# rgcgithub/regenie

Hardware: NVIDIA H100
Metric: step1_level0_snps_per_sec (higher is better)
Workload: dtype int8 Gram + int8 prediction (both exact integer sums) + tf32x3 factorisation + f64 refinement / statistics

## Files before the change

regenie_b200/csrc/bed_kernels.cu:

```cuda
#include "kernels.cuh"

namespace rg {

__device__ __forceinline__ uint32_t plink_to_code(uint32_t v, int ref_first) {
  const uint32_t lut = ref_first ? 0x9Cu : 0x1Eu;
  return (lut >> (2 * v)) & 3u;
}

__global__ void bed_relayout_kernel(const uint8_t* __restrict__ packed, int64_t row_stride, int bs,
                                    const int32_t* __restrict__ file_idx_pad, const int32_t* __restrict__ word_base,
                                    const uint32_t* __restrict__ word_keep, int ref_first,
                                    uint32_t* __restrict__ gp, int64_t words_per_row) {
  const int64_t w = blockIdx.x * (int64_t)blockDim.x + threadIdx.x;
  const int row = blockIdx.y;
  if (w >= words_per_row) return;
  uint32_t out = 0;
  const int base = (row < bs) ? __ldg(word_base + w) : -1;
  if (base >= 0) {
    const uint8_t* p = packed + (int64_t)row * row_stride + (base >> 2);
    const int64_t left = row_stride - (base >> 2);
    uint64_t x = 0;
#pragma unroll
    for (int b = 0; b < 5; ++b)
      if (b < left) x |= (uint64_t)__ldg(p + b) << (8 * b);
    const uint32_t v = (uint32_t)(x >> (2 * (base & 3)));
    const uint32_t H = (v >> 1) & 0x55555555u, Lo = v & 0x55555555u;
    const uint32_t oh = ref_first ? Lo : (~H & 0x55555555u);
    out = ((oh << 1) | (H ^ Lo)) & __ldg(word_keep + w);
  } else if (base == -2) {
    const uint8_t* prow = packed + (int64_t)row * row_stride;
    const int4* fi4 = reinterpret_cast<const int4*>(file_idx_pad + w * 16);
#pragma unroll
    for (int q = 0; q < 4; ++q) {
      const int4 f = __ldg(fi4 + q);
      const int fi[4] = {f.x, f.y, f.z, f.w};
#pragma unroll
      for (int k = 0; k < 4; ++k) {
        uint32_t code = 0;
        if (fi[k] >= 0) {
          const uint32_t b = __ldg(prow + (fi[k] >> 2));
          code = plink_to_code((b >> (2 * (fi[k] & 3))) & 3u, ref_first);
        }
        out |= code << (2 * (q * 4 + k));
      }
    }
  }
  gp[(int64_t)row * words_per_row + w] = out;
}

void launch_bed_relayout(const uint8_t* packed, int64_t row_stride, int bs, int rows_p,
                         const int32_t* file_idx_pad, const int32_t* word_base, const uint32_t* word_keep, int ref_first,
                         uint32_t* gp, int64_t npad,
                         cudaStream_t s) {
  const int64_t wpr = npad / 16;
  dim3 grid((unsigned)ceil_div(wpr, 256), rows_p);
  bed_relayout_kernel<<<grid, 256, 0, s>>>(packed, row_stride, bs, file_idx_pad, word_base, word_keep, ref_first, gp, wpr);
}

}
```

regenie_b200/csrc/context.cuh:

```cuda
#pragma once
#include <map>
#include <memory>

#include "../../include/rg_b200.h"
#include "kernels.cuh"

struct rg_ctx;
namespace rg { void ensure_W(::rg_ctx* h); }

struct rg_ctx {
  int kind = 0;
  int device = 0;
  cudaStream_t stream = nullptr;
  int64_t launches = 0;

  int64_t N = 0, Npad = 0, n_analyzed = 0;
  int C = 0, P = 0, K = 1, R = 0, R1 = 0, loocv = 0;
  int bs_max = 0, rows_p_max = 0, total_blocks = 0, cpp = 0;
  int64_t B = 0;

  std::vector<int64_t> fold_sizes, fold_pad_start, fold_pad_len;
  std::vector<int32_t> pad_of;
  std::vector<int32_t> src_of;
  std::vector<uint8_t> in_analysis;
// ... 127 lines not shown
  rg::DevBuf<double> s2_male_tot;
  int bt_mode = 0, bt_dp = 0, bt_ncol = 0;
  int s2_fcols = 0;
  bool s2_chr_set = false, bt_chr_set = false;
  int s2_last_bs = 0;
  int s2_sums_rows = 0, bt_sums_rows = 0, bt_sums_dp = 0;
  static constexpr int kStageSlots = 4;
  rg::DevBuf<uint8_t> s2_stage[kStageSlots];
  cudaStream_t s2_copy_stream = nullptr;
  cudaEvent_t s2_stage_ev[kStageSlots] = {nullptr, nullptr, nullptr, nullptr};
  bool s2_stage_pending[kStageSlots] = {false, false, false, false};
  rg::DevBuf<uint8_t> probs_dev, miss_dev;
  rg::DevBuf<uint8_t> inflate_comp, inflate_raw;
  rg::DevBuf<uint64_t> inflate_offs;
  rg::DevBuf<int32_t> inflate_status;
  rg::DevBuf<uint8_t> pgen_in, pgen_rows;
  rg::DevBuf<unsigned long long> pgen_err;
  rg::DevBuf<uint32_t> dz;
  bool int_set = false;
  bool s2_dz_qt = false;
  rg::DevBuf<int8_t> int_route;
  int int_K = 0, int_nr = 0, int_nf = 0;
  rg::DevBuf<double> int_F, int_E, int_part, int_sums, int_var, int_meat, int_out;
  rg::DevBuf<uint8_t> int_pow2;
  rg::DevBuf<int32_t> int_status;
  rg::DevBuf<double> bt_F, bt_w, bt_gs, bt_xw, bt_off, bt_coltot, bt_xwy, bt_part, bt_sums, bt_nnz, bt_n510;
  rg::DevBuf<double> bt_xtwg, bt_mu, bt_info, firth_gvec, firth_out, bt_den, bt_phat;
  rg::DevBuf<int8_t> bt_ym, firth_cflag;
  rg::DevBuf<int2> bt_cnt_part;
  rg::DevBuf<int32_t> firth_sel, firth_status;

  bool gram_dense = false;
  int64_t miss_cap = 0;

  int solver_mixed = 1;
  float mx_tol = 1e-9f;
  int64_t mx_blocks = 0, mx_fallbacks = 0;

  bool timing = false;
  cudaEvent_t ev0 = nullptr, ev1 = nullptr;
  std::map<std::string, std::pair<double, int64_t>> timers;
  std::vector<std::tuple<std::string, cudaEvent_t, cudaEvent_t>> pending;
};

namespace rg {
void require_gpu(int device);
void ensure_file_idx(rg_ctx* h, const int32_t* sample_idx);
void flush_timers(rg_ctx* h);
void sync_lanes(rg_ctx* h);
void pgen_check_errors(rg_ctx* h);
}

#define RG_API_BEGIN try {
#define RG_API_END                         \
  }                                        \
  catch (const rg::Error& e) {             \
    rg::set_last_error(e.msg);             \
    return 1;                              \
  }                                        \
  catch (const std::exception& e) {        \
    rg::set_last_error(e.what());          \
    return 1;                              \
  }                                        \
  return 0;
```

regenie_b200/csrc/kernels.cuh:

```cuda
#pragma once
#include "common.cuh"

namespace rg {

constexpr int kMaxFolds = 16;
constexpr int kMaxCov = 64;
constexpr int kMaxRidge = 8;
constexpr int kMaxPhenoTile = 8;
constexpr int kLimbs = 9;
constexpr int kLimbsI8 = 5;
constexpr int kLimbQI8 = 50;

void launch_bed_relayout(const uint8_t* packed, int64_t row_stride, int bs, int rows_p,
                         const int32_t* file_idx_pad, const int32_t* word_base, const uint32_t* word_keep, int ref_first,
                         uint32_t* gp, int64_t npad,
                         cudaStream_t s);

struct SnpFinalizeArgs {
  int bs, rows_p, C, P, K, cpp, loocv;
  long long n_analyzed;
  double numtol;
  const int32_t* cnt_fold;
  const double* sum_fold;
  const double* XtX_f;
  const double* XtY_f;
  double *mu, *inv_sd;
  double* Bv;
  double *Af, *Qf;
  double *gty_f, *rhs;
  unsigned long long* err_slot;
  long long err_base;
};

struct AssembleArgs {
  int bs, rows_p, nC, C, K, R, loocv;
  const float* zz;
  int64_t ldz, zz_fold_stride;
  const double *mu, *inv_sd, *Bv, *Af, *Qf;
  const double* lambda;
  double* cm;
  int64_t cm_stride;
  int ldc;
  float* planes = nullptr;
  float* lplanes = nullptr;
};

void launch_l0_stats(const uint32_t* gp, int64_t npad, const double* xy, int cpp, const int4* chunks,
                     int nchunks, int rows_p, int32_t* cnt_part, double* sum_part, cudaStream_t s);
void launch_l0_fold_reduce(const int32_t* cnt_part, const double* sum_part, int rows_p, int cpp,
                           const int2* fold_chunks, int K, int32_t* cnt_fold, double* sum_fold,
                           cudaStream_t s);
void launch_l0_snp_finalize(const SnpFinalizeArgs& a, cudaStream_t s);
void launch_l0_assemble(const AssembleArgs& a, const double* rhs, int P, int Ppad, int nmat, cudaStream_t s);

void make_gram_tensor_map(CUtensorMap* tm, const uint8_t* z, int64_t npad, int rows2);
constexpr int kStatQ = 14;
constexpr int kStatOnesRow = 126;
void launch_l0_xy_digits(const double* xy, int cpp, int ncol, int64_t npad, const uint8_t* is_real, double* scale,
                         uint8_t* D, cudaStream_t s);
void launch_l0_stats_finish(const float* T, int ldt, int64_t t_fold_stride, const float* zz, int ldz,
                            int64_t zz_fold_stride, int rows_p, int cpp, int ncol, int K, const double* scale,
                            int32_t* cnt_fold, double* sum_fold, cudaStream_t s);
void gram_tile_list(int rows2, std::vector<int2>& tiles);
void launch_gram_wgmma(const CUtensorMap& tm, const CUtensorMap& tmB, const int2* tiles, int ntiles, const int2* fold_k, int K,
                         float* out, int ldo, int64_t fold_stride, float out_scale, cudaStream_t s, int bn = 256);
void launch_gram_gp(const CUtensorMap& tmG, const CUtensorMap* tmD, int rows_p, const int2* tiles, int ntiles,
                    const int2* fold_k, int K, float* out, int ldo, int64_t fold_stride, float out_scale, cudaStream_t s,
                    int bn = 256, const unsigned long long* miss_total = nullptr, int64_t miss_cap = 0,
                    int miss_tile0 = 0);
constexpr float kZScaleGram = 1.f / 64;
constexpr float kZScaleStat = 1.f / 8;
constexpr double kMissSparseRate = 0.015;
void launch_miss_list(const uint32_t* gp, int64_t npad, int rows_p, const int2* fold_k, int K, unsigned long long* total,
                      int64_t cap, int2* seg, int32_t* list, cudaStream_t s);
void launch_miss_transpose(const uint32_t* gp, int64_t npad, int rows_p, const unsigned long long* total, int64_t cap,
                           uint32_t* gt, cudaStream_t s);
void launch_miss_sparse(const uint32_t* gt, int rows_p, const int2* seg, const int32_t* list, int K,
                        const unsigned long long* total, int64_t cap, float* zz, int64_t fold_stride, cudaStream_t s);
void launch_gram_reference(const uint32_t* gp, int64_t npad, int rows_p, int k0, int k1, float* out, int ldo,
                           cudaStream_t s);

void launch_chol_factor(double* cm, int64_t stride, int nC, int n_aug, int batch, double* inv,
                        unsigned long long* err_slot, long long err_base, cudaStream_t s);
void launch_chol_backsolve(double* cm, int64_t stride, int nC, int P, int batch, const double* inv,
                           cudaStream_t s);
int chol_num_launches(int nC);
size_t chol_inv_elems(int nC, int batch);
void launch_chol_rows_backsolve(double* cm, int64_t stride, int nC, int row0, int nrows, int batch,
                                const double* inv, cudaStream_t s);

struct Tf32GemmEpilogue {
  int n;
  int64_t out_mat_stride;
  float* out;
  int mirror;
  int b_cols_local;
  int negate;
  int lower_only;
  const double* cin;
  int64_t cin_mat_stride;
  int cin_ld, cin_mat_div;
  const double* diag_add;
  int diag_mod;
  int c_chunks;
  int c_mat_div;
};
void make_tf32_operand_tensor_map(CUtensorMap* tm, const float* base, int cols, int rows, int batch);
void make_f32_rows_tensor_map(CUtensorMap* tm, const float* base, int cols, int64_t rows, int box_cols, int box_rows);
void launch_tf32x3_gemm(const CUtensorMap& tmA, const CUtensorMap& tmB, const int4* tiles, int ntiles, int batch,
                        const Tf32GemmEpilogue& ep, cudaStream_t s, const CUtensorMap* tmC = nullptr);

// ... 239 lines not shown
```

regenie_b200/csrc/miss_gram.cu:

```cuda
#include "kernels.cuh"

namespace rg {

namespace {

__device__ __forceinline__ uint32_t miss_bits(uint32_t w) { return w & (w >> 1) & 0x55555555u; }

constexpr int kListThreads = 256;
constexpr int kChunkWords = 64;
constexpr int kSparseWarps = 4;
constexpr int kCodeStride = kChunkWords + 1;

}

__global__ void __launch_bounds__(kListThreads)
miss_list_kernel(const uint32_t* __restrict__ gp, int64_t wpr, int rows_p, const int2* __restrict__ fold_k,
                 unsigned long long* __restrict__ total, unsigned long long cap, int2* __restrict__ seg,
                 int32_t* __restrict__ list) {
  const int i = blockIdx.x, f = blockIdx.y;
  const int2 fk = fold_k[f];
  const int64_t w0 = (int64_t)fk.x * (kSamplePad / 16), w1 = (int64_t)(fk.x + fk.y) * (kSamplePad / 16);
  const uint32_t* row = gp + (int64_t)i * wpr;
  __shared__ int warp_cnt[kListThreads / 32];
  __shared__ unsigned long long base_s;
  __shared__ int pos_s;
  int n = 0;
  for (int64_t w = w0 + threadIdx.x; w < w1; w += kListThreads) n += __popc(miss_bits(__ldg(row + w)));
#pragma unroll
  for (int o = 16; o > 0; o >>= 1) n += __shfl_xor_sync(0xffffffffu, n, o);
  if ((threadIdx.x & 31) == 0) warp_cnt[threadIdx.x >> 5] = n;
  __syncthreads();
  if (threadIdx.x == 0) {
    int cnt = 0;
    for (int k = 0; k < kListThreads / 32; ++k) cnt += warp_cnt[k];
    const unsigned long long base = cnt ? atomicAdd(total, (unsigned long long)cnt) : 0ull;
    seg[(int64_t)f * rows_p + i] = make_int2((int)(base + cnt <= cap ? base : 0), base + cnt <= cap ? cnt : 0);
    base_s = base + cnt <= cap ? base : ~0ull;
    pos_s = 0;
  }
  __syncthreads();
  const unsigned long long base = base_s;
  if (base == ~0ull) return;
  for (int64_t w = w0 + threadIdx.x; w < w1; w += kListThreads) {
    uint32_t m = miss_bits(__ldg(row + w));
    if (!m) continue;
    int p = atomicAdd(&pos_s, __popc(m));
    for (; m; m &= m - 1) list[base + p++] = (int32_t)(w * 16 + (__ffs(m) - 1) / 2);
  }
}

__global__ void __launch_bounds__(256)
miss_transpose_kernel(const uint32_t* __restrict__ gp, int64_t wpr, int rows_p,
                      const unsigned long long* __restrict__ total, unsigned long long cap, uint32_t* __restrict__ gt) {
  if (*total > cap) return;
  __shared__ uint32_t t[128][33];
  const int64_t wb = (int64_t)blockIdx.x * 32;
  const int r0 = blockIdx.y * 128;
  for (int k = threadIdx.x; k < 128 * 32; k += 256) {
    const int r = k >> 5, c = k & 31;
    t[r][c] = (wb + c < wpr) ? __ldg(gp + (int64_t)(r0 + r) * wpr + wb + c) : 0u;
  }
  __syncthreads();
  const int gw = rows_p / 16;
#pragma unroll
  for (int q = 0; q < 2; ++q) {
    const int sl = threadIdx.x + 256 * q;
    const int c = sl >> 4, sh = 2 * (sl & 15);
    if (wb + c >= wpr) continue;
    uint32_t o[8];
#pragma unroll
    for (int jw = 0; jw < 8; ++jw) {
      uint32_t v = 0;
#pragma unroll
      for (int r = 0; r < 16; ++r) v |= ((t[jw * 16 + r][c] >> sh) & 3u) << (2 * r);
      o[jw] = v;
    }
    uint4* dst = reinterpret_cast<uint4*>(gt + (wb * 16 + sl) * gw + blockIdx.y * 8);
    dst[0] = make_uint4(o[0], o[1], o[2], o[3]);
    dst[1] = make_uint4(o[4], o[5], o[6], o[7]);
  }
}

__global__ void __launch_bounds__(32 * kSparseWarps)
miss_sparse_kernel(const uint32_t* __restrict__ gt, int rows_p, const int2* __restrict__ seg,
                   const int32_t* __restrict__ list, const unsigned long long* __restrict__ total,
                   unsigned long long cap, float* __restrict__ zz, int64_t fold_stride) {
  if (*total > cap) return;
  __shared__ uint32_t acc_s[kSparseWarps][2][16 * kCodeStride];
  __shared__ int smp_s[kSparseWarps][128];
  const int warp = threadIdx.x >> 5, lane = threadIdx.x & 31;
  const int i = blockIdx.x * kSparseWarps + warp, f = blockIdx.y;
  uint32_t* sG = acc_s[warp][0];
  uint32_t* sM = acc_s[warp][1];
  int* sSmp = smp_s[warp];
  const int2 sg = seg[(int64_t)f * rows_p + i];
  const int32_t* lst = list + sg.x;
  const int cnt = sg.y;
  const int gw = rows_p / 16;
  const int r = rows_p + i;
  const int colmax = min(2 * rows_p, 256 * ((r / 128) / 2 + 1));
  float* out = zz + (int64_t)f * fold_stride + (int64_t)r * (2 * rows_p);
  constexpr int off[4] = {0, 2, 1, 3};

  for (int w0 = 0; w0 < gw; w0 += kChunkWords) {
    for (int k = lane; k < 16 * kCodeStride; k += 32) { sG[k] = 0; sM[k] = 0; }
    __syncwarp();
    for (int b0 = 0; b0 < cnt; b0 += 126) {
      const int n = min(cnt - b0, 126);
#pragma unroll
      for (int k = 0; k < 4; ++k) sSmp[32 * k + lane] = 32 * k + lane < n ? __ldg(lst + b0 + 32 * k + lane) : -1;
      __syncwarp();
      uint32_t g8[2][4] = {}, m8[2][4] = {};
      for (int g0 = 0; g0 < n; g0 += 7) {
        uint32_t g4[2][2] = {}, m4[2][2] = {};
        int smp[7];
#pragma unroll
        for (int u = 0; u < 7; ++u) smp[u] = sSmp[g0 + u];
#pragma unroll
        for (int u = 0; u < 7; ++u) {
#pragma unroll
          for (int h = 0; h < 2; ++h) {
            const int w = w0 + lane + 32 * h;
            const uint32_t x = (smp[u] >= 0 && w < gw) ? __ldg(gt + (int64_t)smp[u] * gw + w) : 0u;
            const uint32_t m = miss_bits(x);
            const uint32_t gx = x & ~(m * 3u);
            g4[h][0] += gx & 0x33333333u;
            g4[h][1] += (gx >> 2) & 0x33333333u;
            m4[h][0] += m & 0x11111111u;
            m4[h][1] += (m >> 2) & 0x11111111u;
          }
        }
#pragma unroll
        for (int h = 0; h < 2; ++h) {
          g8[h][0] += g4[h][0] & 0x0F0F0F0Fu;
          g8[h][1] += (g4[h][0] >> 4) & 0x0F0F0F0Fu;
          g8[h][2] += g4[h][1] & 0x0F0F0F0Fu;
          g8[h][3] += (g4[h][1] >> 4) & 0x0F0F0F0Fu;
          m8[h][0] += m4[h][0] & 0x0F0F0F0Fu;
          m8[h][1] += (m4[h][0] >> 4) & 0x0F0F0F0Fu;
          m8[h][2] += m4[h][1] & 0x0F0F0F0Fu;
          m8[h][3] += (m4[h][1] >> 4) & 0x0F0F0F0Fu;
        }
      }
#pragma unroll
      for (int h = 0; h < 2; ++h)
#pragma unroll
        for (int q = 0; q < 4; ++q)
#pragma unroll
          for (int b = 0; b < 4; ++b) {
            const int k = (4 * b + off[q]) * kCodeStride + lane + 32 * h;
            sG[k] += (g8[h][q] >> (8 * b)) & 0xFFu;
            sM[k] += (m8[h][q] >> (8 * b)) & 0xFFu;
          }
      __syncwarp();
    }
    __syncwarp();
    const int j0 = 16 * w0, j1 = min(rows_p, 16 * (w0 + kChunkWords));
    for (int j = j0 + lane; j < j1; j += 32) {
      const int k = (j & 15) * kCodeStride + (j >> 4) - w0;
      out[j] = (float)sG[k];
      if (rows_p + j < colmax) out[rows_p + j] = (float)sM[k];
    }
    __syncwarp();
  }
}

void launch_miss_list(const uint32_t* gp, int64_t npad, int rows_p, const int2* fold_k, int K, unsigned long long* total,
                      int64_t cap, int2* seg, int32_t* list, cudaStream_t s) {
  RG_CUDA(cudaMemsetAsync(total, 0, sizeof(unsigned long long), s));
  miss_list_kernel<<<dim3(rows_p, K), kListThreads, 0, s>>>(gp, npad / 16, rows_p, fold_k, total, (unsigned long long)cap,
                                                            seg, list);
}

void launch_miss_transpose(const uint32_t* gp, int64_t npad, int rows_p, const unsigned long long* total, int64_t cap,
                           uint32_t* gt, cudaStream_t s) {
  const int64_t wpr = npad / 16;
  miss_transpose_kernel<<<dim3((unsigned)ceil_div(wpr, 32), rows_p / 128), 256, 0, s>>>(gp, wpr, rows_p, total,
                                                                                          (unsigned long long)cap, gt);
}

void launch_miss_sparse(const uint32_t* gt, int rows_p, const int2* seg, const int32_t* list, int K,
                        const unsigned long long* total, int64_t cap, float* zz, int64_t fold_stride, cudaStream_t s) {
  miss_sparse_kernel<<<dim3(rows_p / kSparseWarps, K), 32 * kSparseWarps, 0, s>>>(gt, rows_p, seg, list, total,
                                                                                   (unsigned long long)cap, zz, fold_stride);
}

}
```

regenie_b200/csrc/rg_api.cu:

```cuda
#include <string.h>

#include <algorithm>
#include <mutex>

#include "context.cuh"

namespace rg {

static thread_local std::string g_last_error;
void set_last_error(const std::string& m) { g_last_error = m; }

bool is_device_pointer(const void* p) {
  cudaPointerAttributes at;
  cudaError_t e = cudaPointerGetAttributes(&at, p);
  if (e != cudaSuccess) {
    cudaGetLastError();
    return false;
  }
  return at.type == cudaMemoryTypeDevice || at.type == cudaMemoryTypeManaged;
}

void copy_to_device(void* dst, const void* src, size_t bytes, cudaStream_t stream) {
  if (bytes == 0) return;
  RG_CUDA(cudaMemcpyAsync(dst, src, bytes, cudaMemcpyDefault, stream));
// ... 150 lines not shown
  h->fold_k.alloc(K);
  h->XtX_f.alloc(XtX.size());
  h->XtY_f.alloc(XtY.size());
  RG_CUDA(cudaMemcpyAsync(h->xy.p, xy.data(), xy.size() * 8, cudaMemcpyHostToDevice, s));
  RG_CUDA(cudaMemcpyAsync(h->mask.p, maskp.data(), maskp.size(), cudaMemcpyHostToDevice, s));
  RG_CUDA(cudaMemcpyAsync(h->is_real.p, is_real.data(), is_real.size(), cudaMemcpyHostToDevice, s));
  RG_CUDA(cudaMemcpyAsync(h->tile_fold.p, tile_fold.data(), tile_fold.size() * 4, cudaMemcpyHostToDevice, s));
  RG_CUDA(cudaMemcpyAsync(h->chunks.p, chunks.data(), chunks.size() * sizeof(int4), cudaMemcpyHostToDevice, s));
  RG_CUDA(cudaMemcpyAsync(h->fold_chunks.p, fold_chunks.data(), K * sizeof(int2), cudaMemcpyHostToDevice, s));
  RG_CUDA(cudaMemcpyAsync(h->fold_k.p, fold_k.data(), K * sizeof(int2), cudaMemcpyHostToDevice, s));
  RG_CUDA(cudaMemcpyAsync(h->XtX_f.p, XtX.data(), XtX.size() * 8, cudaMemcpyHostToDevice, s));
  RG_CUDA(cudaMemcpyAsync(h->XtY_f.p, XtY.data(), XtY.size() * 8, cudaMemcpyHostToDevice, s));
  {
    int64_t max_fold = 0;
    for (int f = 0; f < K; ++f) max_fold = std::max(max_fold, h->fold_pad_len[f]);
    const char* e = getenv("RG_B200_STATS");
    h->stats_tc = !(e && std::string(e) == "f64") && max_fold * 30 < (1ll << 24);
    if (h->stats_tc) {
      const int ngroups = (int)ceil_div(C + P, kStatQ);
      h->stat_drows = ngroups * 128;
      h->xyD.alloc((size_t)h->stat_drows * h->Npad);
      h->xy_scale.alloc(h->cpp);
      RG_CUDA(cudaMemsetAsync(h->xyD.p, 0, (size_t)h->stat_drows * h->Npad, s));
      launch_l0_xy_digits(h->xy.p, h->cpp, C + P, h->Npad, h->is_real.p, h->xy_scale.p, h->xyD.p, s);
      make_gram_tensor_map(&h->tmD, h->xyD.p, h->Npad, h->stat_drows);
    }
  }
  {
    const char* e = getenv("RG_B200_GRAM");
    const std::string mode = e ? e : "";
    h->gram_dense = mode == "dense";
    const double rate = mode == "sparse" ? 1.0 : kMissSparseRate;
    h->miss_cap = std::min<int64_t>((int64_t)(rate * h->bs_max * h->n_analyzed), INT32_MAX);
  }
  RG_CUDA(cudaStreamSynchronize(s));
}

static void build_file_idx(rg_ctx* h, const int32_t* sample_idx_host) {
  std::vector<int32_t> fi(h->Npad, -1);
  for (int64_t t = 0; t < h->Npad; ++t) {
    const int32_t s = h->src_of[t];
    if (s < 0 || !h->in_analysis[s]) continue;
    fi[t] = sample_idx_host ? sample_idx_host[s] : s;
  }
  const int64_t nw = h->Npad / 16;
  std::vector<int32_t> wb(nw, -1);
  std::vector<uint32_t> wk(nw, 0);
  for (int64_t w = 0; w < nw; ++w) {
    int32_t base = -1;
    bool contiguous = true;
    for (int j = 0; j < 16; ++j) {
      const int32_t f = fi[w * 16 + j];
      if (f < 0) continue;
      wk[w] |= 3u << (2 * j);
      if (base == -1) base = f - j;
      else if (f - j != base) contiguous = false;
    }
    wb[w] = (wk[w] == 0) ? -1 : ((contiguous && base >= 0) ? base : -2);
  }
  h->file_idx_pad.alloc(h->Npad);
  h->word_base.alloc(nw);
  h->word_keep.alloc(nw);
  RG_CUDA(cudaMemcpyAsync(h->word_base.p, wb.data(), nw * 4, cudaMemcpyHostToDevice, h->stream));
  RG_CUDA(cudaMemcpyAsync(h->word_keep.p, wk.data(), nw * 4, cudaMemcpyHostToDevice, h->stream));
  RG_CUDA(cudaMemcpyAsync(h->file_idx_pad.p, fi.data(), fi.size() * 4, cudaMemcpyHostToDevice, h->stream));
  RG_CUDA(cudaStreamSynchronize(h->stream));
// ... 277 lines not shown
    {
      ScopedTimer t(h, "h2d", cs);
      copy_to_device(buf.p, packed, (size_t)bs * row_stride, cs);
    }
    RG_CUDA(cudaEventRecord(L.h2d_done, cs));
    L.h2d_recorded = true;
    RG_CUDA(cudaStreamWaitEvent(s, L.h2d_done, 0));
    packed_d = buf.p;
  }
  resolve_lane(h, L);

  L.gp.alloc((size_t)h->rows_p_max * (Npad / 16));
  L.zz.alloc((size_t)K * 4 * h->rows_p_max * h->rows_p_max);
  L.cnt_part.alloc((size_t)h->nchunks * h->rows_p_max * 4);
  L.sum_part.alloc((size_t)h->nchunks * h->rows_p_max * 2 * h->cpp);
  L.cnt_fold.alloc((size_t)K * h->rows_p_max * 4);
  L.sum_fold.alloc((size_t)K * h->rows_p_max * 2 * h->cpp);
  L.mu.alloc(h->rows_p_max);
  L.inv_sd.alloc(h->rows_p_max);
  L.Bv.alloc((size_t)h->rows_p_max * C);
  L.Af.alloc((size_t)K * h->rows_p_max * C);
  L.Qf.alloc((size_t)K * h->rows_p_max * C);
  L.gty_f.alloc((size_t)K * h->rows_p_max * P);
  L.rhs.alloc((size_t)K * h->rows_p_max * P);
  const int Kg = h->loocv ? 1 : K;
  L.gam.alloc((size_t)Kg * h->rows_p_max * Qp);
  L.gmu.alloc((size_t)Kg * h->rows_p_max * Qp);
  L.cvec.alloc((size_t)Kg * Qp * C);
  L.part.alloc((size_t)d.ntiles_s * Qp * 2);
  L.mean_invsd.alloc((size_t)2 * Qp);

  {
    ScopedTimer t(h, "bed_relayout", s);
    launch_bed_relayout(packed_d, row_stride, bs, rows_p, h->file_idx_pad.p, h->word_base.p, h->word_keep.p, ref_first, L.gp.p, Npad, s);
    if (staged >= 0) {
      if (!L.relayout_done[staged]) RG_CUDA(cudaEventCreateWithFlags(&L.relayout_done[staged], cudaEventDisableTiming));
      RG_CUDA(cudaEventRecord(L.relayout_done[staged], s));
      L.relayout_recorded[staged] = true;
    }
  }
  h->launches += 1;

  auto snp_finalize = [&]() {
    SnpFinalizeArgs a;
    a.bs = bs; a.rows_p = rows_p; a.C = C; a.P = P; a.K = K; a.cpp = h->cpp; a.loocv = h->loocv;
    a.n_analyzed = h->n_analyzed; a.numtol = 1e-6;
    a.cnt_fold = L.cnt_fold.p; a.sum_fold = L.sum_fold.p; a.XtX_f = h->XtX_f.p; a.XtY_f = h->XtY_f.p;
    a.mu = L.mu.p; a.inv_sd = L.inv_sd.p; a.Bv = L.Bv.p; a.Af = L.Af.p; a.Qf = L.Qf.p;
    a.gty_f = L.gty_f.p; a.rhs = L.rhs.p; a.err_slot = h->err_slot.p;
    a.err_base = (long long)block_id * h->bs_max;
    launch_l0_snp_finalize(a, s);
    h->launches += 1;
  };
  if (!h->stats_tc) {
    ScopedTimer t(h, "l0_stats", s);
    launch_l0_stats(L.gp.p, Npad, h->xy.p, h->cpp, h->chunks.p, h->nchunks, rows_p, L.cnt_part.p,
                    L.sum_part.p, s);
    launch_l0_fold_reduce(L.cnt_part.p, L.sum_part.p, rows_p, h->cpp, h->fold_chunks.p, K,
                          L.cnt_fold.p, L.sum_fold.p, s);
    snp_finalize();
    h->launches += 2;
  }

  {
    const rg_ctx::TileList& tl =
        cached_tiles(h->tile_lists, rows_p, [&](std::vector<int2>& tiles) { gram_tile_list(2 * rows_p, tiles); });
    const int64_t zz_stride = (int64_t)4 * rows_p * rows_p;
    ScopedTimer t(h, "gram_wgmma", s);
    if (h->gram_dense) {
      launch_gram_gp(gp_map(h, L, rows_p), nullptr, rows_p, tl.buf.p, tl.count, h->fold_k.p, K,
                     L.zz.p, 2 * rows_p, zz_stride, kZScaleGram, s);
      h->launches += 1;
    } else {
      L.miss_total.alloc(1);
      L.miss_seg.alloc((size_t)K * h->rows_p_max);
      L.miss_list.alloc((size_t)std::max<int64_t>(h->miss_cap, 1));
      L.gt.alloc((size_t)Npad * (h->rows_p_max / 16));
      launch_miss_list(L.gp.p, Npad, rows_p, h->fold_k.p, K, L.miss_total.p, h->miss_cap, L.miss_seg.p, L.miss_list.p, s);
      launch_miss_transpose(L.gp.p, Npad, rows_p, L.miss_total.p, h->miss_cap, L.gt.p, s);
      launch_gram_gp(gp_map(h, L, rows_p), nullptr, rows_p, tl.buf.p, tl.count, h->fold_k.p, K,
                     L.zz.p, 2 * rows_p, zz_stride, kZScaleGram, s, 256, L.miss_total.p, h->miss_cap, rows_p / 128);
      launch_miss_sparse(L.gt.p, rows_p, L.miss_seg.p, L.miss_list.p, K, L.miss_total.p, h->miss_cap, L.zz.p, zz_stride, s);
      h->launches += 5;
    }
    L.last_gram_dense = h->gram_dense;
  }
  if (h->stats_tc) {
    ScopedTimer t(h, "l0_stats", s);
    const int stat_bn = (h->stat_drows % 256 == 0) ? 256 : 128;
    const rg_ctx::TileList& tl = cached_tiles(h->stat_tile_lists, rows_p, [&](std::vector<int2>& tiles) {
      for (int nj = 0; nj < h->stat_drows / stat_bn; ++nj)
        for (int mi = 0; mi < 2 * rows_p / 128; ++mi) tiles.push_back(make_int2(mi, nj));
    });
    L.tstat.alloc((size_t)K * 2 * h->rows_p_max * h->stat_drows);
    const int64_t tfs = (int64_t)2 * rows_p * h->stat_drows;
    launch_gram_gp(gp_map(h, L, rows_p), &h->tmD, rows_p, tl.buf.p, tl.count, h->fold_k.p,
                   K, L.tstat.p, h->stat_drows, tfs, kZScaleStat, s, stat_bn);
    launch_l0_stats_finish(L.tstat.p, h->stat_drows, tfs, L.zz.p, 2 * rows_p, (int64_t)4 * rows_p * rows_p, rows_p,
                           h->cpp, C + P, K, h->xy_scale.p, L.cnt_fold.p, L.sum_fold.p, s);
    snp_finalize();
    h->launches += 2;
  }

  const int mx_n = (!h->loocv && h->solver_mixed) ? MixedSolver::dim_for(bs) : 0;
  L.last_mx_n = mx_n;
  if (mx_n > 0) {
    enqueue_solve_mixed(h, L, d, mx_n, s);
    enqueue_predict(h, L, d, L.mx_x.p, (int64_t)mx_pp(P) * mx_n, mx_n, 0, s);
    RG_CUDA(cudaMemcpyAsync(L.mx_fail_host, L.mx_fail.p, sizeof(unsigned int), cudaMemcpyDeviceToHost, s));
    RG_CUDA(cudaEventRecord(L.mx_ev, s));
    L.mx_pending = true; L.mx_bs = bs; L.mx_block_id = block_id;
    h->mx_blocks += 1;
    return;
  }
  enqueue_solve_f64(h, L, d, s);
  if (!h->loocv) enqueue_predict(h, L, d, L.cm.p, (int64_t)d.n_aug * d.nC, d.nC, d.nC, s);
// ... 125 lines not shown
  if (n == "inv_sd") return dev_view(L.inv_sd.p, (size_t)rp * 8);
  if (n == "Bv") return dev_view(L.Bv.p, (size_t)rp * h->C * 8);
  if (n == "gty_f") return dev_view(L.gty_f.p, (size_t)h->K * rp * h->P * 8);
  if (n == "rhs") return dev_view(L.rhs.p, (size_t)h->K * rp * h->P * 8);
  if (n == "cm") return dev_view(L.cm.p, (size_t)h->last_nmat * h->last_n_aug * h->last_nC * 8);
  if (n == "mean_invsd") return dev_view(L.mean_invsd.p, (size_t)2 * h->R * h->P * 8);
  if (n == "wraw") return dev_view(L.wraw.p, (size_t)h->P * h->R * h->Npad * 8);
  if (n == "gam" || n == "gmu" || n == "cvec") {
    const size_t Kg = h->loocv ? 1 : h->K, Qp = (size_t)round_up(h->R * h->P, predict_qt());
    const DevBuf<double>& b = n == "gam" ? L.gam : n == "gmu" ? L.gmu : L.cvec;
    return dev_view(b.p, (n == "cvec" ? Kg * Qp * h->C : Kg * rp * Qp) * 8);
  }
  if (n == "cnt_fold") return dev_view(L.cnt_fold.p, (size_t)h->K * rp * 4 * 4);
  if (n == "sum_fold") return dev_view(L.sum_fold.p, (size_t)h->K * rp * 2 * h->cpp * 8);
  if (n == "paths") {
    const int64_t v[3] = {h->stats_tc ? 1 : 0, L.last_pred_i8, L.last_mx_n};
    return host_view(v, 3);
  }
  if (n == "dims") {
    const int64_t v[8] = {h->Npad, rp, h->last_nC, h->last_n_aug, h->last_nmat, h->K, h->cpp, h->nchunks};
    return host_view(v, 8);
  }
  if (n == "gram_path") {
    int64_t v[3] = {0, -1, h->miss_cap};
    if (!L.last_gram_dense) {
      RG_CHECK(L.miss_total.p, "debug buffer not filled yet: gram_path");
      unsigned long long tot = 0;
      RG_CUDA(cudaStreamSynchronize(L.stream));
      RG_CUDA(cudaMemcpy(&tot, L.miss_total.p, sizeof(tot), cudaMemcpyDeviceToHost));
      v[0] = (int64_t)tot <= h->miss_cap ? 1 : 0;
      v[1] = (int64_t)tot;
    }
    return host_view(v, 3);
  }
  if (n == "pad_of") return host_view(h->pad_of.data(), h->N);
  if (n == "zz_ref") {
    RG_CHECK(L.gp.p, "debug buffer not filled yet: gp");
    const size_t per = (size_t)4 * rp * rp;
    DevBuf<float> ref;
    ref.alloc(per * h->K);
    RG_CUDA(cudaMemsetAsync(ref.p, 0, per * h->K * 4, h->stream));
    for (int f = 0; f < h->K; ++f)
      launch_gram_reference(L.gp.p, h->Npad, rp, (int)h->fold_pad_start[f], (int)(h->fold_pad_start[f] + h->fold_pad_len[f]),
                            ref.p + per * f, 2 * rp, h->stream);
    std::vector<float> v(per * h->K);
    RG_CUDA(cudaMemcpyAsync(v.data(), ref.p, v.size() * 4, cudaMemcpyDeviceToHost, h->stream));
    RG_CUDA(cudaStreamSynchronize(h->stream));
    return host_view(v.data(), v.size());
  }
  throw Error{"unknown debug buffer: " + n};
}

static DebugView debug_view(rg_ctx* h, const std::string& n, int64_t max_bytes) {
  if (n == "pgen_rows") {
    const DevBuf<uint8_t>& r = h->kind == 1 && !h->lanes.empty() ? h->lanes[h->next_lane]->packed_dev : h->pgen_rows;
    RG_CHECK(r.p, "pgen_rows: no rg_pgen_decode has filled it");
    return dev_view(r.p, std::min<size_t>(r.n, (size_t)std::max<int64_t>(max_bytes, 0)));
  }
  if (h->kind == 2) return s2_debug_view(h, n);
  if (n.compare(0, 3, "l1_") == 0) return l1_debug_view(h, n);
  return l0_debug_view(h, n);
}

static int64_t copy_debug_view(const DebugView& v, const std::string& n, void* out, int64_t max_bytes) {
  RG_CHECK(v.dev || !v.host.empty(), "debug buffer not filled yet: " + n);
  RG_CHECK((int64_t)v.bytes <= max_bytes, "buffer too small for " + n + ": it needs " + std::to_string(v.bytes) + " bytes");
// ... 410 lines not shown
```

Before: 968,800.

## Fuse missing-genotype list and transpose into tiled BED relayout kernel

The BED relayout kernel now works on 128-row by 32-word tiles held in shared memory. In the sparse-missing path the same kernel also builds per-tile missing-sample lists, using a block scan and one atomic per tile, and writes the bit-transposed genotype matrix. This removes the separate miss_list and miss_transpose kernels, which each re-read the whole genotype buffer. The sparse Gram kernel now gathers its list entries across per-tile segments, which adds per-batch scan overhead in exchange for fewer passes over global memory.

Result: faster. 1.006 million (median of 6 runs) (+3.9%).

```diff
diff --git a/regenie_b200/csrc/bed_kernels.cu b/regenie_b200/csrc/bed_kernels.cu
--- a/regenie_b200/csrc/bed_kernels.cu
+++ b/regenie_b200/csrc/bed_kernels.cu
@@ -7,13 +7,10 @@
   return (lut >> (2 * v)) & 3u;
 }
 
-__global__ void bed_relayout_kernel(const uint8_t* __restrict__ packed, int64_t row_stride, int bs,
-                                    const int32_t* __restrict__ file_idx_pad, const int32_t* __restrict__ word_base,
-                                    const uint32_t* __restrict__ word_keep, int ref_first,
-                                    uint32_t* __restrict__ gp, int64_t words_per_row) {
-  const int64_t w = blockIdx.x * (int64_t)blockDim.x + threadIdx.x;
-  const int row = blockIdx.y;
-  if (w >= words_per_row) return;
+__device__ __forceinline__ uint32_t bed_word(const uint8_t* __restrict__ packed, int64_t row_stride, int row, int bs,
+                                             int64_t w, const int32_t* __restrict__ file_idx_pad,
+                                             const int32_t* __restrict__ word_base,
+                                             const uint32_t* __restrict__ word_keep, int ref_first) {
   uint32_t out = 0;
   const int base = (row < bs) ? __ldg(word_base + w) : -1;
   if (base >= 0) {
@@ -45,16 +42,131 @@
       }
     }
   }
-  gp[(int64_t)row * words_per_row + w] = out;
+  return out;
+}
+
+namespace {
+
+constexpr int kTileRows = 128;
+constexpr int kTileWords = 32;
+constexpr int kRelayoutThreads = 256;
+
+__device__ __forceinline__ int warp_inclusive_scan(int v, int lane) {
+#pragma unroll
+  for (int o = 1; o < 32; o <<= 1) {
+    const int u = __shfl_up_sync(0xffffffffu, v, o);
+    if (lane >= o) v += u;
+  }
+  return v;
+}
+
+}
+
+template <bool kMiss>
+__global__ void __launch_bounds__(kRelayoutThreads)
+bed_relayout_kernel(const uint8_t* __restrict__ packed, int64_t row_stride, int bs,
+                    const int32_t* __restrict__ file_idx_pad, const int32_t* __restrict__ word_base,
+                    const uint32_t* __restrict__ word_keep, int ref_first, uint32_t* __restrict__ gp, int64_t wpr,
+                    BedMissOut mo) {
+  const int r0 = blockIdx.y * kTileRows;
+  const int lane = threadIdx.x & 31, warp = threadIdx.x >> 5;
+  int64_t w0;
+  int nw;
+  if constexpr (kMiss) {
+    const int4 ct = __ldg(mo.ctile + blockIdx.x);
+    w0 = ct.x;
+    nw = ct.y;
+  } else {
+    w0 = (int64_t)blockIdx.x * kTileWords;
+    nw = (int)(wpr - w0 < kTileWords ? wpr - w0 : kTileWords);
+  }
+  __shared__ uint32_t t[kMiss ? kTileRows : 1][kTileWords + 1];
+#pragma unroll 2
+  for (int r = warp; r < kTileRows; r += kRelayoutThreads / 32) {
+    const int row = r0 + r;
+    uint32_t v = 0;
+    if (lane < nw) {
+      v = bed_word(packed, row_stride, row, bs, w0 + lane, file_idx_pad, word_base, word_keep, ref_first);
+      gp[(int64_t)row * wpr + w0 + lane] = v;
+    }
+    if constexpr (kMiss) t[r][lane] = v;
+  }
+  if constexpr (kMiss) {
+    __shared__ int cnt_s[kTileRows], pre_s[kTileRows];
+    __shared__ unsigned long long base_s;
+    __syncthreads();
+    for (int r = warp; r < kTileRows; r += kRelayoutThreads / 32) {
+      const int n = __reduce_add_sync(0xffffffffu, (unsigned)__popc(miss_bits(t[r][lane])));
+      if (lane == 0) cnt_s[r] = n;
+    }
+    __syncthreads();
+    if (warp == 0) {
+      int c[4], sum = 0;
+#pragma unroll
+      for (int q = 0; q < 4; ++q) { c[q] = cnt_s[4 * lane + q]; sum += c[q]; }
+      const int inc = warp_inclusive_scan(sum, lane);
+      int p = inc - sum;
+#pragma unroll
+      for (int q = 0; q < 4; ++q) { pre_s[4 * lane + q] = p; p += c[q]; }
+      if (lane == 31) {
+        const unsigned long long base = inc ? atomicAdd(mo.total, (unsigned long long)inc) : 0ull;
+        base_s = base + inc <= mo.cap ? base : ~0ull;
+      }
+    }
+    __syncthreads();
+    const unsigned long long base = base_s;
+    if (base == ~0ull) return;
+    if (threadIdx.x < kTileRows)
+      mo.seg[(int64_t)(r0 + threadIdx.x) * mo.nct + blockIdx.x] =
+          make_int2((int)(base + pre_s[threadIdx.x]), cnt_s[threadIdx.x]);
+    for (int r = warp; r < kTileRows; r += kRelayoutThreads / 32) {
+      if (!cnt_s[r]) continue;
+      uint32_t m = miss_bits(t[r][lane]);
+      const int n = __popc(m);
+      int64_t p = (int64_t)base + pre_s[r] + warp_inclusive_scan(n, lane) - n;
+      for (; m; m &= m - 1) mo.list[p++] = (int32_t)((w0 + lane) * 16 + (__ffs(m) - 1) / 2);
+    }
+    const int gw = mo.rows_p / 16;
+    const int jw = lane & 7, c = 4 * warp + (lane >> 3);
+    if (c < nw) {
+      uint32_t a[16];
+#pragma unroll
+      for (int r = 0; r < 16; ++r) a[r] = t[16 * jw + r][c];
+      uint32_t m = 0x0000FFFFu;
+#pragma unroll
+      for (int j = 8; j != 0; j >>= 1, m ^= m << (2 * j))
+#pragma unroll
+        for (int k = 0; k < 16; k = (k + j + 1) & ~j) {
+          const uint32_t x = ((a[k] >> (2 * j)) ^ a[k + j]) & m;
+          a[k] ^= x << (2 * j);
+          a[k + j] ^= x;
+        }
+      uint32_t* dst = mo.gt + (w0 + c) * 16 * gw + blockIdx.y * 8 + jw;
+#pragma unroll
+      for (int q = 0; q < 16; ++q) dst[(int64_t)q * gw] = a[q];
+    }
+  }
 }
 
 void launch_bed_relayout(const uint8_t* packed, int64_t row_stride, int bs, int rows_p,
                          const int32_t* file_idx_pad, const int32_t* word_base, const uint32_t* word_keep, int ref_first,
                          uint32_t* gp, int64_t npad,
                          cudaStream_t s) {
+  RG_CHECK(rows_p % kTileRows == 0, "bed_relayout: rows_p must be a multiple of 128");
   const int64_t wpr = npad / 16;
-  dim3 grid((unsigned)ceil_div(wpr, 256), rows_p);
-  bed_relayout_kernel<<<grid, 256, 0, s>>>(packed, row_stride, bs, file_idx_pad, word_base, word_keep, ref_first, gp, wpr);
+  dim3 grid((unsigned)ceil_div(wpr, kTileWords), (unsigned)(rows_p / kTileRows));
+  bed_relayout_kernel<false><<<grid, kRelayoutThreads, 0, s>>>(packed, row_stride, bs, file_idx_pad, word_base,
+                                                               word_keep, ref_first, gp, wpr, BedMissOut{});
+}
+
+void launch_bed_relayout_miss(const uint8_t* packed, int64_t row_stride, int bs, int rows_p,
+                              const int32_t* file_idx_pad, const int32_t* word_base, const uint32_t* word_keep,
+                              int ref_first, uint32_t* gp, int64_t npad, const BedMissOut& mo, cudaStream_t s) {
+  RG_CHECK(rows_p % kTileRows == 0 && mo.rows_p == rows_p, "bed_relayout_miss: rows_p must be a multiple of 128");
+  RG_CUDA(cudaMemsetAsync(mo.total, 0, sizeof(unsigned long long), s));
+  dim3 grid((unsigned)mo.nct, (unsigned)(rows_p / kTileRows));
+  bed_relayout_kernel<true><<<grid, kRelayoutThreads, 0, s>>>(packed, row_stride, bs, file_idx_pad, word_base,
+                                                              word_keep, ref_first, gp, npad / 16, mo);
 }
 
 }
diff --git a/regenie_b200/csrc/context.cuh b/regenie_b200/csrc/context.cuh
--- a/regenie_b200/csrc/context.cuh
+++ b/regenie_b200/csrc/context.cuh
@@ -183,6 +183,10 @@
 
   bool gram_dense = false;
   int64_t miss_cap = 0;
+  int miss_nct = 0;
+  std::vector<int4> miss_ctile_host;
+  rg::DevBuf<int4> miss_ctile;
+  rg::DevBuf<int2> miss_fold_ct;
 
   int solver_mixed = 1;
   float mx_tol = 1e-9f;
diff --git a/regenie_b200/csrc/kernels.cuh b/regenie_b200/csrc/kernels.cuh
--- a/regenie_b200/csrc/kernels.cuh
+++ b/regenie_b200/csrc/kernels.cuh
@@ -11,10 +11,24 @@
 constexpr int kLimbsI8 = 5;
 constexpr int kLimbQI8 = 50;
 
+__device__ __forceinline__ uint32_t miss_bits(uint32_t w) { return w & (w >> 1) & 0x55555555u; }
+struct BedMissOut {
+  const int4* ctile = nullptr;
+  int nct = 0;
+  int rows_p = 0;
+  unsigned long long* total = nullptr;
+  unsigned long long cap = 0;
+  int2* seg = nullptr;
+  int32_t* list = nullptr;
+  uint32_t* gt = nullptr;
+};
 void launch_bed_relayout(const uint8_t* packed, int64_t row_stride, int bs, int rows_p,
                          const int32_t* file_idx_pad, const int32_t* word_base, const uint32_t* word_keep, int ref_first,
                          uint32_t* gp, int64_t npad,
                          cudaStream_t s);
+void launch_bed_relayout_miss(const uint8_t* packed, int64_t row_stride, int bs, int rows_p,
+                              const int32_t* file_idx_pad, const int32_t* word_base, const uint32_t* word_keep,
+                              int ref_first, uint32_t* gp, int64_t npad, const BedMissOut& mo, cudaStream_t s);
 
 struct SnpFinalizeArgs {
   int bs, rows_p, C, P, K, cpp, loocv;
@@ -71,12 +85,9 @@
 constexpr float kZScaleGram = 1.f / 64;
 constexpr float kZScaleStat = 1.f / 8;
 constexpr double kMissSparseRate = 0.015;
-void launch_miss_list(const uint32_t* gp, int64_t npad, int rows_p, const int2* fold_k, int K, unsigned long long* total,
-                      int64_t cap, int2* seg, int32_t* list, cudaStream_t s);
-void launch_miss_transpose(const uint32_t* gp, int64_t npad, int rows_p, const unsigned long long* total, int64_t cap,
-                           uint32_t* gt, cudaStream_t s);
-void launch_miss_sparse(const uint32_t* gt, int rows_p, const int2* seg, const int32_t* list, int K,
-                        const unsigned long long* total, int64_t cap, float* zz, int64_t fold_stride, cudaStream_t s);
+void launch_miss_sparse(const uint32_t* gt, int rows_p, const int2* seg, int nct, const int2* fold_ct,
+                        const int32_t* list, int K, const unsigned long long* total, int64_t cap, float* zz,
+                        int64_t fold_stride, cudaStream_t s);
 void launch_gram_reference(const uint32_t* gp, int64_t npad, int rows_p, int k0, int k1, float* out, int ldo,
                            cudaStream_t s);
 
diff --git a/regenie_b200/csrc/miss_gram.cu b/regenie_b200/csrc/miss_gram.cu
--- a/regenie_b200/csrc/miss_gram.cu
+++ b/regenie_b200/csrc/miss_gram.cu
@@ -4,87 +4,50 @@
 
 namespace {
 
-__device__ __forceinline__ uint32_t miss_bits(uint32_t w) { return w & (w >> 1) & 0x55555555u; }
-
-constexpr int kListThreads = 256;
 constexpr int kChunkWords = 64;
 constexpr int kSparseWarps = 4;
 constexpr int kCodeStride = kChunkWords + 1;
+constexpr int kBatch = 126;
+
+__device__ __forceinline__ int miss_fill_batch(const int2* __restrict__ sg, int& ct, int ct1, int& used,
+                                               const int32_t* __restrict__ list, int* smp, int lane) {
+  int n = 0;
+  while (n < kBatch && ct < ct1) {
+    int2 e = ct + lane < ct1 ? __ldg(sg + ct + lane) : make_int2(0, 0);
+    if (lane == 0) { e.x += used; e.y -= used; }
+    int inc = e.y;
+#pragma unroll
+    for (int o = 1; o < 32; o <<= 1) {
+      const int u = __shfl_up_sync(0xffffffffu, inc, o);
+      if (lane >= o) inc += u;
+    }
+    const int room = kBatch - n, exc = inc - e.y;
+    const int take = max(0, min(e.y, room - exc));
+    for (int k = 0; k < take; ++k) smp[n + exc + k] = __ldg(list + e.x + k);
+    const int all = __shfl_sync(0xffffffffu, inc, 31);
+    if (all <= room) {
+      n += all;
+      ct = min(ct + 32, ct1);
+      used = 0;
+    } else {
+      const int l = __ffs(__ballot_sync(0xffffffffu, inc > room)) - 1;
+      used = (l == 0 ? used : 0) + __shfl_sync(0xffffffffu, take, l);
+      ct += l;
+      n = kBatch;
+    }
+  }
+  for (int k = n + lane; k < 128; k += 32) smp[k] = -1;
+  __syncwarp();
+  return n;
+}
 
 }
 
-__global__ void __launch_bounds__(kListThreads)
-miss_list_kernel(const uint32_t* __restrict__ gp, int64_t wpr, int rows_p, const int2* __restrict__ fold_k,
-                 unsigned long long* __restrict__ total, unsigned long long cap, int2* __restrict__ seg,
-                 int32_t* __restrict__ list) {
-  const int i = blockIdx.x, f = blockIdx.y;
-  const int2 fk = fold_k[f];
-  const int64_t w0 = (int64_t)fk.x * (kSamplePad / 16), w1 = (int64_t)(fk.x + fk.y) * (kSamplePad / 16);
-  const uint32_t* row = gp + (int64_t)i * wpr;
-  __shared__ int warp_cnt[kListThreads / 32];
-  __shared__ unsigned long long base_s;
-  __shared__ int pos_s;
-  int n = 0;
-  for (int64_t w = w0 + threadIdx.x; w < w1; w += kListThreads) n += __popc(miss_bits(__ldg(row + w)));
-#pragma unroll
-  for (int o = 16; o > 0; o >>= 1) n += __shfl_xor_sync(0xffffffffu, n, o);
-  if ((threadIdx.x & 31) == 0) warp_cnt[threadIdx.x >> 5] = n;
-  __syncthreads();
-  if (threadIdx.x == 0) {
-    int cnt = 0;
-    for (int k = 0; k < kListThreads / 32; ++k) cnt += warp_cnt[k];
-    const unsigned long long base = cnt ? atomicAdd(total, (unsigned long long)cnt) : 0ull;
-    seg[(int64_t)f * rows_p + i] = make_int2((int)(base + cnt <= cap ? base : 0), base + cnt <= cap ? cnt : 0);
-    base_s = base + cnt <= cap ? base : ~0ull;
-    pos_s = 0;
-  }
-  __syncthreads();
-  const unsigned long long base = base_s;
-  if (base == ~0ull) return;
-  for (int64_t w = w0 + threadIdx.x; w < w1; w += kListThreads) {
-    uint32_t m = miss_bits(__ldg(row + w));
-    if (!m) continue;
-    int p = atomicAdd(&pos_s, __popc(m));
-    for (; m; m &= m - 1) list[base + p++] = (int32_t)(w * 16 + (__ffs(m) - 1) / 2);
-  }
-}
-
-__global__ void __launch_bounds__(256)
-miss_transpose_kernel(const uint32_t* __restrict__ gp, int64_t wpr, int rows_p,
-                      const unsigned long long* __restrict__ total, unsigned long long cap, uint32_t* __restrict__ gt) {
-  if (*total > cap) return;
-  __shared__ uint32_t t[128][33];
-  const int64_t wb = (int64_t)blockIdx.x * 32;
-  const int r0 = blockIdx.y * 128;
-  for (int k = threadIdx.x; k < 128 * 32; k += 256) {
-    const int r = k >> 5, c = k & 31;
-    t[r][c] = (wb + c < wpr) ? __ldg(gp + (int64_t)(r0 + r) * wpr + wb + c) : 0u;
-  }
-  __syncthreads();
-  const int gw = rows_p / 16;
-#pragma unroll
-  for (int q = 0; q < 2; ++q) {
-    const int sl = threadIdx.x + 256 * q;
-    const int c = sl >> 4, sh = 2 * (sl & 15);
-    if (wb + c >= wpr) continue;
-    uint32_t o[8];
-#pragma unroll
-    for (int jw = 0; jw < 8; ++jw) {
-      uint32_t v = 0;
-#pragma unroll
-      for (int r = 0; r < 16; ++r) v |= ((t[jw * 16 + r][c] >> sh) & 3u) << (2 * r);
-      o[jw] = v;
-    }
-    uint4* dst = reinterpret_cast<uint4*>(gt + (wb * 16 + sl) * gw + blockIdx.y * 8);
-    dst[0] = make_uint4(o[0], o[1], o[2], o[3]);
-    dst[1] = make_uint4(o[4], o[5], o[6], o[7]);
-  }
-}
-
 __global__ void __launch_bounds__(32 * kSparseWarps)
-miss_sparse_kernel(const uint32_t* __restrict__ gt, int rows_p, const int2* __restrict__ seg,
-                   const int32_t* __restrict__ list, const unsigned long long* __restrict__ total,
-                   unsigned long long cap, float* __restrict__ zz, int64_t fold_stride) {
+miss_sparse_kernel(const uint32_t* __restrict__ gt, int rows_p, const int2* __restrict__ seg, int nct,
+                   const int2* __restrict__ fold_ct, const int32_t* __restrict__ list,
+                   const unsigned long long* __restrict__ total, unsigned long long cap, float* __restrict__ zz,
+                   int64_t fold_stride) {
   if (*total > cap) return;
   __shared__ uint32_t acc_s[kSparseWarps][2][16 * kCodeStride];
   __shared__ int smp_s[kSparseWarps][128];
@@ -93,9 +56,8 @@
   uint32_t* sG = acc_s[warp][0];
   uint32_t* sM = acc_s[warp][1];
   int* sSmp = smp_s[warp];
-  const int2 sg = seg[(int64_t)f * rows_p + i];
-  const int32_t* lst = list + sg.x;
-  const int cnt = sg.y;
+  const int2* sg = seg + (int64_t)i * nct;
+  const int2 fct = fold_ct[f];
   const int gw = rows_p / 16;
   const int r = rows_p + i;
   const int colmax = min(2 * rows_p, 256 * ((r / 128) / 2 + 1));
@@ -105,11 +67,10 @@
   for (int w0 = 0; w0 < gw; w0 += kChunkWords) {
     for (int k = lane; k < 16 * kCodeStride; k += 32) { sG[k] = 0; sM[k] = 0; }
     __syncwarp();
-    for (int b0 = 0; b0 < cnt; b0 += 126) {
-      const int n = min(cnt - b0, 126);
-#pragma unroll
-      for (int k = 0; k < 4; ++k) sSmp[32 * k + lane] = 32 * k + lane < n ? __ldg(lst + b0 + 32 * k + lane) : -1;
-      __syncwarp();
+    int ct = fct.x, used = 0;
+    for (;;) {
+      const int n = miss_fill_batch(sg, ct, fct.y, used, list, sSmp, lane);
+      if (n == 0) break;
       uint32_t g8[2][4] = {}, m8[2][4] = {};
       for (int g0 = 0; g0 < n; g0 += 7) {
         uint32_t g4[2][2] = {}, m4[2][2] = {};
@@ -165,24 +126,11 @@
   }
 }
 
-void launch_miss_list(const uint32_t* gp, int64_t npad, int rows_p, const int2* fold_k, int K, unsigned long long* total,
-                      int64_t cap, int2* seg, int32_t* list, cudaStream_t s) {
-  RG_CUDA(cudaMemsetAsync(total, 0, sizeof(unsigned long long), s));
-  miss_list_kernel<<<dim3(rows_p, K), kListThreads, 0, s>>>(gp, npad / 16, rows_p, fold_k, total, (unsigned long long)cap,
-                                                            seg, list);
-}
-
-void launch_miss_transpose(const uint32_t* gp, int64_t npad, int rows_p, const unsigned long long* total, int64_t cap,
-                           uint32_t* gt, cudaStream_t s) {
-  const int64_t wpr = npad / 16;
-  miss_transpose_kernel<<<dim3((unsigned)ceil_div(wpr, 32), rows_p / 128), 256, 0, s>>>(gp, wpr, rows_p, total,
-                                                                                          (unsigned long long)cap, gt);
-}
-
-void launch_miss_sparse(const uint32_t* gt, int rows_p, const int2* seg, const int32_t* list, int K,
-                        const unsigned long long* total, int64_t cap, float* zz, int64_t fold_stride, cudaStream_t s) {
-  miss_sparse_kernel<<<dim3(rows_p / kSparseWarps, K), 32 * kSparseWarps, 0, s>>>(gt, rows_p, seg, list, total,
-                                                                                   (unsigned long long)cap, zz, fold_stride);
+void launch_miss_sparse(const uint32_t* gt, int rows_p, const int2* seg, int nct, const int2* fold_ct,
+                        const int32_t* list, int K, const unsigned long long* total, int64_t cap, float* zz,
+                        int64_t fold_stride, cudaStream_t s) {
+  miss_sparse_kernel<<<dim3(rows_p / kSparseWarps, K), 32 * kSparseWarps, 0, s>>>(
+      gt, rows_p, seg, nct, fold_ct, list, total, (unsigned long long)cap, zz, fold_stride);
 }
 
 }
diff --git a/regenie_b200/csrc/rg_api.cu b/regenie_b200/csrc/rg_api.cu
--- a/regenie_b200/csrc/rg_api.cu
+++ b/regenie_b200/csrc/rg_api.cu
@@ -206,6 +206,21 @@
     h->gram_dense = mode == "dense";
     const double rate = mode == "sparse" ? 1.0 : kMissSparseRate;
     h->miss_cap = std::min<int64_t>((int64_t)(rate * h->bs_max * h->n_analyzed), INT32_MAX);
+    std::vector<int2> fold_ct(K);
+    h->miss_ctile_host.clear();
+    for (int f = 0; f < K; ++f) {
+      fold_ct[f].x = (int)h->miss_ctile_host.size();
+      const int64_t w1 = (h->fold_pad_start[f] + h->fold_pad_len[f]) / 16;
+      for (int64_t w = h->fold_pad_start[f] / 16; w < w1; w += 32)
+        h->miss_ctile_host.push_back(make_int4((int)w, (int)std::min<int64_t>(32, w1 - w), f, 0));
+      fold_ct[f].y = (int)h->miss_ctile_host.size();
+    }
+    h->miss_nct = (int)h->miss_ctile_host.size();
+    h->miss_ctile.alloc(h->miss_nct);
+    h->miss_fold_ct.alloc(K);
+    RG_CUDA(cudaMemcpyAsync(h->miss_ctile.p, h->miss_ctile_host.data(), h->miss_nct * sizeof(int4),
+                            cudaMemcpyHostToDevice, s));
+    RG_CUDA(cudaMemcpyAsync(h->miss_fold_ct.p, fold_ct.data(), K * sizeof(int2), cudaMemcpyHostToDevice, s));
   }
   RG_CUDA(cudaStreamSynchronize(s));
 }
@@ -549,7 +564,22 @@
 
   {
     ScopedTimer t(h, "bed_relayout", s);
-    launch_bed_relayout(packed_d, row_stride, bs, rows_p, h->file_idx_pad.p, h->word_base.p, h->word_keep.p, ref_first, L.gp.p, Npad, s);
+    if (h->gram_dense) {
+      launch_bed_relayout(packed_d, row_stride, bs, rows_p, h->file_idx_pad.p, h->word_base.p, h->word_keep.p,
+                          ref_first, L.gp.p, Npad, s);
+    } else {
+      L.miss_total.alloc(1);
+      L.miss_seg.alloc((size_t)h->rows_p_max * h->miss_nct);
+      L.miss_list.alloc((size_t)std::max<int64_t>(h->miss_cap, 1));
+      L.gt.alloc((size_t)Npad * (h->rows_p_max / 16));
+      BedMissOut mo;
+      mo.ctile = h->miss_ctile.p; mo.nct = h->miss_nct; mo.rows_p = rows_p;
+      mo.total = L.miss_total.p; mo.cap = (unsigned long long)h->miss_cap;
+      mo.seg = L.miss_seg.p; mo.list = L.miss_list.p; mo.gt = L.gt.p;
+      launch_bed_relayout_miss(packed_d, row_stride, bs, rows_p, h->file_idx_pad.p, h->word_base.p, h->word_keep.p,
+                               ref_first, L.gp.p, Npad, mo, s);
+      h->launches += 1;
+    }
     if (staged >= 0) {
       if (!L.relayout_done[staged]) RG_CUDA(cudaEventCreateWithFlags(&L.relayout_done[staged], cudaEventDisableTiming));
       RG_CUDA(cudaEventRecord(L.relayout_done[staged], s));
@@ -589,16 +619,11 @@
                      L.zz.p, 2 * rows_p, zz_stride, kZScaleGram, s);
       h->launches += 1;
     } else {
-      L.miss_total.alloc(1);
-      L.miss_seg.alloc((size_t)K * h->rows_p_max);
-      L.miss_list.alloc((size_t)std::max<int64_t>(h->miss_cap, 1));
-      L.gt.alloc((size_t)Npad * (h->rows_p_max / 16));
-      launch_miss_list(L.gp.p, Npad, rows_p, h->fold_k.p, K, L.miss_total.p, h->miss_cap, L.miss_seg.p, L.miss_list.p, s);
-      launch_miss_transpose(L.gp.p, Npad, rows_p, L.miss_total.p, h->miss_cap, L.gt.p, s);
       launch_gram_gp(gp_map(h, L, rows_p), nullptr, rows_p, tl.buf.p, tl.count, h->fold_k.p, K,
                      L.zz.p, 2 * rows_p, zz_stride, kZScaleGram, s, 256, L.miss_total.p, h->miss_cap, rows_p / 128);
-      launch_miss_sparse(L.gt.p, rows_p, L.miss_seg.p, L.miss_list.p, K, L.miss_total.p, h->miss_cap, L.zz.p, zz_stride, s);
-      h->launches += 5;
+      launch_miss_sparse(L.gt.p, rows_p, L.miss_seg.p, h->miss_nct, h->miss_fold_ct.p, L.miss_list.p, K,
+                         L.miss_total.p, h->miss_cap, L.zz.p, zz_stride, s);
+      h->launches += 2;
     }
     L.last_gram_dense = h->gram_dense;
   }
@@ -790,6 +815,12 @@
       v[1] = (int64_t)tot;
     }
     return host_view(v, 3);
+  }
+  if (n == "miss_ctile") return host_view(h->miss_ctile_host.data(), h->miss_ctile_host.size());
+  if (n == "miss_seg" || n == "miss_list") {
+    RG_CHECK(!L.last_gram_dense && L.miss_seg.p, "no missing lists for the last block: " + n);
+    if (n == "miss_seg") return dev_view(L.miss_seg.p, (size_t)rp * h->miss_nct * sizeof(int2));
+    return dev_view(L.miss_list.p, (size_t)std::max<int64_t>(h->miss_cap, 1) * 4);
   }
   if (n == "pad_of") return host_view(h->pad_of.data(), h->N);
   if (n == "zz_ref") {
```
